# sash-a/CleanRL.jl

Measured on AMD Instinct MI355X. Metric: env-steps/sec (whole node), CartPole PPO num_envs=65536 at 1/2/4/8 GPUs, higher is better.
Workload: dtype f32 (64x64 products as fp16x2 split operands — hi + lo in f16, >= 22 significant bits — 3 f16 MFMAs per product, f32 accumulate; measured against a Float64 product on the headline's own operands this is as close as a plain f32 FMA chain: profiles/r06_product_error.json)

## Files before the change

### cleanrl.jl_amd/_lib.py

```python
import ctypes as C
import os

import numpy as np

_HERE = os.path.dirname(os.path.abspath(__file__))
LIB_PATH = os.environ.get("CRL_LIB_PATH") or os.path.join(_HERE, "libcleanrl_hip.so")


class CrlError(RuntimeError):
    pass


class CrlConfig(C.Structure):
    _fields_ = [
        ("total_timesteps", C.c_int64), ("num_steps", C.c_int32), ("num_envs", C.c_int32),
        ("num_minibatches", C.c_int32), ("update_epochs", C.c_int32), ("lr", C.c_float), ("gamma", C.c_float),
        ("gae_lambda", C.c_float), ("clip_coef", C.c_float), ("ent_coeff", C.c_float), ("v_coef", C.c_float),
        ("normalize_advantages", C.c_int32), ("clip_value_loss", C.c_int32), ("anneal_lr", C.c_int32),
        ("obs_dim", C.c_int32), ("n_act", C.c_int32), ("hidden", C.c_int32), ("gae_mode", C.c_int32),
        ("env_kind", C.c_int32), ("stale_obs", C.c_int32), ("env_id_offset", C.c_int32), ("shuffle_mode", C.c_int32),
        ("seed", C.c_uint64),
    ]


# ... 39 lines not shown
        return {n: getattr(self, n) for n, _ in self._fields_}


EXPORTS = [
    "crl_version", "crl_last_error", "crl_device_count", "crl_ppo_create", "crl_ppo_destroy", "crl_ppo_param_count",
    "crl_sync", "crl_ppo_write", "crl_ppo_read", "crl_policy_act", "crl_logprob_actions", "crl_gae",
    "crl_rollout_store", "crl_env_reset", "crl_rollout_run", "crl_episode_stats_read", "crl_compute_gae",
    "crl_shuffle", "crl_adv_stats", "crl_ppo_update_minibatch", "crl_ppo_iterate", "crl_ppo_iteration",
    "crl_comm_unique_id", "crl_comm_init", "crl_comm_init_external", "crl_comm_peer_export", "crl_comm_peer_attach", "crl_adv_stats_local", "crl_adv_stats_finish",
    "crl_prof_enable", "crl_prof_read", "crl_prof_reset", "crl_ppo_exact_reruns", "crl_episode_ring_enable",
    "crl_episode_ring_read", "crl_comm_destroy", "crl_ppo_set_option", "crl_ppo_get_option", "crl_ppo_option_name", "crl_ppo_option_count", "crl_gae_bench", "crl_gae_opt",
    "crl_a2c_create", "crl_a2c_destroy", "crl_a2c_param_count", "crl_a2c_write_params", "crl_a2c_read_params",
    "crl_a2c_read_env", "crl_a2c_read_buffer", "crl_a2c_run_until_update", "crl_a2c_discounted_future_rewards",
    "crl_dqn_create", "crl_dqn_destroy", "crl_dqn_write_params", "crl_dqn_read_params", "crl_dqn_status_read", "crl_dqn_run",
    "crl_dqn_q_values",
    "crl_make_actor_critic", "crl_ppo_init_params", "crl_a2c_init_params", "crl_dqn_make_nn", "crl_dqn_init_params", "crl_comm_info", "crl_clock_probe", "crl_product_probe", "crl_ppo_iterate_async", "crl_ppo_drain",
    "crl_env_step", "crl_ppo_evaluate", "crl_ppo_diagnose",
    "crl_ppo_stream", "crl_rollout_act_device", "crl_rollout_record_device", "crl_env_step_device", "crl_ppo_update",
]

DQN_PARAM_COUNT = 10934


class CrlDQNConfig(C.Structure):
    _fields_ = [("log_frequency", C.c_int64), ("total_timesteps", C.c_int64), ("buffer_size", C.c_int64), ("min_buff_size", C.c_int64),
                ("lr", C.c_double), ("train_freq", C.c_int64), ("target_net_freq", C.c_int64), ("batch_size", C.c_int64),
                ("gamma", C.c_double), ("epsilon_start", C.c_double), ("epsilon_end", C.c_double), ("epsilon_duration", C.c_double),
                ("max_steps", C.c_int32), ("pad", C.c_int32), ("seed", C.c_uint64)]


class CrlDQNEpisode(C.Structure):
# ... 109 lines not shown
    L.crl_make_actor_critic.argtypes = [C.c_int32, C.c_int32, C.c_int32, C.c_uint64, fp, C.c_size_t]
    L.crl_ppo_init_params.argtypes = [vp, C.c_uint64]
    L.crl_a2c_init_params.argtypes = [vp, C.c_uint64]
    L.crl_dqn_make_nn.argtypes = [C.c_uint64, fp, C.c_size_t]
    L.crl_dqn_init_params.argtypes = [vp, C.c_uint64]
    L.crl_comm_info.argtypes = [C.c_char_p, C.c_size_t, ip]
    L.crl_clock_probe.argtypes = [C.c_int32, C.c_double, dp, dp, dp]
    L.crl_ppo_iterate_async.argtypes = [vp, C.POINTER(CrlIterationReport), C.POINTER(CrlStats), C.POINTER(CrlEpisodeRecord), C.c_int32]
    L.crl_ppo_drain.argtypes = [vp, C.POINTER(CrlIterationReport), C.POINTER(CrlStats), C.POINTER(CrlEpisodeRecord), C.c_int32]
    L.crl_ppo_stream.argtypes = [vp, C.POINTER(vp)]
    L.crl_rollout_act_device.argtypes = [vp, C.c_int32, vp, vp, vp, vp]
    L.crl_rollout_record_device.argtypes = [vp, C.c_int32, vp, vp, vp, vp]
    L.crl_env_step_device.argtypes = [vp, vp, C.c_uint64, vp, vp, vp, vp]
    L.crl_ppo_update.argtypes = [vp, C.POINTER(CrlStats)]
    L.crl_product_probe.argtypes = [C.c_int32, C.c_int32, fp, fp, C.c_int32, C.c_int32, C.c_int32, C.c_int32, C.c_float, C.c_float, fp, fp]
    for name in EXPORTS:
        if name not in ("crl_version", "crl_last_error"):
            getattr(L, name).restype = C.c_int32
    _lib = L
    return L


def check(rc):
    if rc != 0:
        raise CrlError(load().crl_last_error().decode("utf-8", "replace"))


def device_count():
    n = C.c_int32(0)
    rc = load().crl_device_count(C.byref(n))
# ... 76 lines not shown
            self.close()
        except Exception:
            pass


def product_probe(flavour, A, B, chunks=1, scale_a=1.0, scale_b=1.0, col_scale=None, device=0):
    A = np.ascontiguousarray(A, np.float32); B = np.ascontiguousarray(B, np.float32)
    rows, K = A.shape; cols = B.shape[0]
    out = np.zeros((chunks, cols, rows), np.float32)
    cs = None if col_scale is None else np.ascontiguousarray(col_scale, np.float32)
    check(load().crl_product_probe(device, flavour, _ptr(A, C.c_float), _ptr(B, C.c_float), rows, cols, K, chunks, scale_a, scale_b,
                                   None if cs is None else _ptr(cs, C.c_float), _ptr(out, C.c_float)))
    return out


def clock_probe(device=0, span_ms=5.0):
    med, lo, hi = C.c_double(0), C.c_double(0), C.c_double(0)
    check(load().crl_clock_probe(device, span_ms, C.byref(med), C.byref(lo), C.byref(hi)))
    return med.value, lo.value, hi.value


def comm_info():
    buf = C.create_string_buffer(4096)
    ver = C.c_int32(0)
    check(load().crl_comm_info(buf, len(buf), C.byref(ver)))
    return buf.value.decode("utf-8", "replace"), int(ver.value)


def make_actor_critic_host(obs_dim, n_act, hidden, seed=0):
    n = 2 * (hidden * obs_dim + hidden + hidden * hidden + hidden) + n_act * hidden + n_act + hidden + 1
# ... 431 lines not shown
```

### cleanrl.jl_amd/csrc/mlp_x2.hpp

```cpp
#pragma once
#include "common.hpp"
#include "mlp_x3.hpp"

namespace crl {

typedef _Float16 f16x8 __attribute__((ext_vector_type(8)));
typedef _Float16 f16x2 __attribute__((ext_vector_type(2)));

constexpr float X2_ACT_SCALE = 16384.0f;
constexpr float X2_W_SCALE = 256.0f;
constexpr float X2_W_LIMIT = 255.0f;
constexpr float X2_W_SMALL = 0.00048828125f;
constexpr float X2_FWD_UNSCALE = 1.0f / (16384.0f * 256.0f);

struct P2 { f16x8 hi, lo; };

__device__ __forceinline__ P2 split2(const float (&x)[8]) {
  P2 p;
#pragma unroll
  for (int q = 0; q < 4; ++q) {
    f32x2 v; v[0] = x[2 * q]; v[1] = x[2 * q + 1];
    const f16x2 h = __builtin_convertvector(v, f16x2);
    f32x2 r;
    const uint32_t hb = __builtin_bit_cast(uint32_t, h);
    asm("v_fma_mix_f32 %0, %1, -1.0, %2 op_sel_hi:[1,0,0]" : "=v"(r[0]) : "v"(hb), "v"(v[0]));
    asm("v_fma_mix_f32 %0, %1, -1.0, %2 op_sel:[1,0,0] op_sel_hi:[1,0,0]" : "=v"(r[1]) : "v"(hb), "v"(v[1]));
    const f16x2 l = __builtin_convertvector(r, f16x2);
    p.hi[2 * q] = h[0]; p.hi[2 * q + 1] = h[1];
    p.lo[2 * q] = l[0]; p.lo[2 * q + 1] = l[1];
  }
  return p;
}

__device__ __forceinline__ f32x16 mfma_f16(f16x8 a, f16x8 b, f32x16 c) {
  return __builtin_amdgcn_mfma_f32_32x32x16_f16(a, b, c, 0, 0, 0);
}
__device__ __forceinline__ f32x16 mfma_x2(const P2& a, const P2& b, f32x16 c) {
  c = mfma_f16(a.lo, b.hi, c);
  c = mfma_f16(a.hi, b.lo, c);
  c = mfma_f16(a.hi, b.hi, c);
  return c;
}

template <int D, int NOUT, bool BWD = true>
struct NetImageX2 {
  static constexpr int PIECE = 2048;
  static constexpr int WF2H = 0;
  static constexpr int WB2H = WF2H + 2 * PIECE;
  static constexpr int WF1 = WB2H + (BWD ? 2 * PIECE : 0);
  static constexpr int B1C = WF1 + 2 * (D / 2) * 64;
  static constexpr int B2C = B1C + 64;
  static constexpr int W3 = B2C + 64;
  static constexpr int B3 = W3 + NOUT * 64;
  static constexpr int SIZE = ((B3 + NOUT + 3) / 4) * 4;
};

template <int D, int NOUT, bool BWD = true>
__device__ __forceinline__ bool stage_net_x2(float* img, const float* __restrict__ p, int tid, int nthreads, int* lds_flag) {
  using I = NetImageX2<D, NOUT, BWD>;
  using P = NetParams<D, NOUT>;
  _Float16* wf = reinterpret_cast<_Float16*>(img + I::WF2H);
  _Float16* wb = reinterpret_cast<_Float16*>(img + I::WB2H);
  if (tid == 0) *lds_flag = 0;
  __syncthreads();
  bool bad = false, big = false;
  for (int idx = tid; idx < 4096; idx += nthreads) {
    const int j = idx & 7, lane = (idx >> 3) & 63, ks = (idx >> 9) & 3, mo = idx >> 11;
    const int i = lane & 31, hf = lane >> 5;
    const int row = 32 * mo + i, k = kmap(ks, j, hf);
    {
      const float w0 = p[P::W2 + row + H * k];
      bad |= !(__builtin_fabsf(w0) < X2_W_LIMIT);
      big |= __builtin_fabsf(w0) >= X2_W_SMALL;
      const float w = w0 * X2_W_SCALE;
      const _Float16 h = (_Float16)w;
      wf[idx] = h; wf[4096 + idx] = (_Float16)(w - (float)h);
    }
    if (BWD) {
// ... 7 lines not shown
    int i = lane & 31, hf = lane >> 5;
    img[I::WF1 + idx] = p[P::W1 + (32 * mo + i) + H * (2 * ks + hf)] * TWO_LOG2E;
  }
  for (int idx = tid; idx < 64; idx += nthreads) {
    int r = idx & 15, mo = (idx >> 4) & 1, hf = idx >> 5;
    int row = 32 * mo + rowmap(r, hf);
    img[I::B1C + idx] = p[P::B1 + row] * TWO_LOG2E;
    img[I::B2C + idx] = p[P::B2 + row] * (X2_ACT_SCALE * X2_W_SCALE);
  }
  for (int idx = tid; idx < NOUT * 64; idx += nthreads) {
    int q = idx & 31, hf = (idx >> 5) & 1, a = idx >> 6;
    int mt = q >> 4, r = q & 15;
    img[I::W3 + idx] = p[P::W3 + a + NOUT * (32 * mt + rowmap(r, hf))];
  }
  for (int idx = tid; idx < NOUT; idx += nthreads) img[I::B3 + idx] = p[P::B3 + idx];
  if (bad) atomicOr(lds_flag, 1);
  if (big) atomicOr(lds_flag, 2);
  __syncthreads();
  return *lds_flag == 2;
}

__device__ __forceinline__ P2 load_wfrag2(const float* piece0, int mo, int ks, int lane) {
  const f16x8* q = reinterpret_cast<const f16x8*>(piece0) + ((mo * 4 + ks) * 64 + lane);
  P2 a;
  a.hi = q[0]; a.lo = q[512];
  return a;
}

__device__ __forceinline__ void dense64_x2(const float* wimg, const f32x16 (&xs)[2], f32x16& acc0, f32x16& acc1, int lane) {
#pragma unroll
  for (int ks = 0; ks < 4; ++ks) {
    float xb[8];
#pragma unroll
    for (int j = 0; j < 8; ++j) xb[j] = xs[ks >> 1][8 * (ks & 1) + j];
    const P2 b = split2(xb);
    acc0 = mfma_x2(load_wfrag2(wimg, 0, ks, lane), b, acc0);
    acc1 = mfma_x2(load_wfrag2(wimg, 1, ks, lane), b, acc1);
  }
}

template <int D, int NOUT, bool BWD = true>
__device__ __forceinline__ void mlp_forward_x2(const float* img, const float (&x)[D], f32x16 (&h1s)[2], f32x16 (&h2)[2],
                                               float (&out)[NOUT], int lane) {
  using I = NetImageX2<D, NOUT, BWD>;
  const int hf = lane >> 5;
  f32x16 a0 = load16(img + I::B1C + hf * 32);
  f32x16 a1 = load16(img + I::B1C + hf * 32 + 16);
#pragma unroll
  for (int ks = 0; ks < D / 2; ++ks) {
    const float b = hf ? x[2 * ks + 1] : x[2 * ks];
    a0 = mfma32(img[I::WF1 + (0 * (D / 2) + ks) * 64 + lane], b, a0);
    a1 = mfma32(img[I::WF1 + (1 * (D / 2) + ks) * 64 + lane], b, a1);
  }
#pragma unroll
  for (int r = 0; r < 16; ++r) { h1s[0][r] = tanh_exp2_arg(a0[r], X2_ACT_SCALE); h1s[1][r] = tanh_exp2_arg(a1[r], X2_ACT_SCALE); }
  a0 = load16(img + I::B2C + hf * 32);
  a1 = load16(img + I::B2C + hf * 32 + 16);
  dense64_x2(img + I::WF2H, h1s, a0, a1, lane);
#pragma unroll
  for (int r = 0; r < 16; ++r) {
    h2[0][r] = tanh_exp2(a0[r], TWO_LOG2E * X2_FWD_UNSCALE, 1.0f); h2[1][r] = tanh_exp2(a1[r], TWO_LOG2E * X2_FWD_UNSCALE, 1.0f);
  }
#pragma unroll
  for (int a = 0; a < NOUT; ++a) {
    const f32x4* w = reinterpret_cast<const f32x4*>(img + I::W3 + a * 64 + hf * 32);
    float acc = 0.0f;
#pragma unroll
    for (int q = 0; q < 8; ++q) {
// ... 47 lines not shown
```

### cleanrl.jl_amd/csrc/policy.hip

```cpp
#include <cstdlib>

#include "common.hpp"
#include "env.hpp"
#include "mlp_x3.hpp"
#include "mlp_x2.hpp"
#include "ppo_ctx.hpp"
#include "rollout_env.hpp"

namespace crl {

template <int D, int A>
__global__ void __launch_bounds__(256) policy_act_kernel(const float* __restrict__ params, const float* __restrict__ obs,
                                                         const double* __restrict__ u, int n, int32_t* __restrict__ action,
                                                         float* __restrict__ logprob, float* __restrict__ value) {
  using IA = NetImage<D, A, false>;
  extern __shared__ __attribute__((aligned(16))) float smem[];
  float* imgA = smem;
  float* imgC = smem + IA::SIZE;
  stage_net<D, A, false>(imgA, params, threadIdx.x, blockDim.x);
  stage_net<D, 1, false>(imgC, params + NetParams<D, A>::SIZE, threadIdx.x, blockDim.x);
  __syncthreads();
  const int lane = threadIdx.x & 63, wave = threadIdx.x >> 6, j = lane & 31, hf = lane >> 5;
  const int wpb = blockDim.x >> 6;
  for (int tile = blockIdx.x * wpb + wave; tile * TILE < n; tile += gridDim.x * wpb) {
// ... 164 lines not shown
  using L = RolloutLds1<A>;
  extern __shared__ __attribute__((aligned(16))) float smem[];
  float* imgA0 = smem + L::IMG_A;
  float* imgC0 = smem + L::IMG_C;
  bool cx2 = CX2;
  stage_net_x3<D, A, false>(imgA0, a.params, threadIdx.x, blockDim.x);
  if (CX2) {
    int* flag = reinterpret_cast<int*>(smem + L::FLAG);
    if (!stage_net_x2<D, 1, false>(imgC0, a.params + NetParams<D, A>::SIZE, threadIdx.x, blockDim.x, flag)) {
      if (threadIdx.x == 0 && blockIdx.x == 0) a.range_err[0] = 1.0;
      cx2 = false;
    }
  }
  if (!cx2) stage_net_x3<D, 1, false>(imgC0, a.params + NetParams<D, A>::SIZE, threadIdx.x, blockDim.x);
  __syncthreads();
  const DevCfg& c = a.c;
  const int lane = threadIdx.x & 63, wave = threadIdx.x >> 6, j = lane & 31, hf = lane >> 5;
  const int wpb = blockDim.x >> 6;
  const int e = (blockIdx.x * wpb + wave) * TILE + j;
  const bool ok = e < c.nt;
  const bool writer = ok && hf == 0;
  const int ee = ok ? e : 0;
  const uint32_t gid = c.env_id_offset + (uint32_t)ee;

  EnvOwner env;
  env_owner_load(env, a, ee);

  if (__builtin_amdgcn_readfirstlane(wave) >= 4) {
    for (int i = 0; i < a.stagger; ++i) __builtin_amdgcn_s_sleep(16);
  }

  for (int step = 0; step < c.k; ++step) {
    const uint64_t gstep = a.iteration * (uint64_t)c.k + (uint64_t)step;
    const size_t b = (size_t)ee + (size_t)c.nt * step;
    f32x16 h1[2], h2[2];
    float z[A], v[1];
    int lds_off = 0;
    asm volatile("" : "+v"(lds_off));
    const float* imgA = imgA0 + lds_off;
    const float* imgC = imgC0 + lds_off;
    const float cx[4] = {env.co[0], env.co[1], env.co[2], env.co[3]};
    mlp_forward_x3<D, A, false>(imgA, cx, h1, h2, z, lane);
    float lpa;
    const int act = env_owner_sample<A>(z, u53(philox_env(c.seed, gid, gstep, 0)), lpa);
    if (CX2 && cx2) mlp_forward_x2<D, 1, false>(imgC, cx, h1, h2, v, lane);
    else mlp_forward_x3<D, 1, false>(imgC, cx, h1, h2, v, lane);
    if (writer) a.value[b] = v[0];
    env_owner_advance(env, a, act, lpa, gid, gstep, step, b, writer);
  }
  if (writer) env_owner_store(env, a, e);
  if (a.fuse_gae) {
    __builtin_amdgcn_fence(__ATOMIC_RELEASE, "workgroup");
    __builtin_amdgcn_fence(__ATOMIC_ACQUIRE, "workgroup");
  }
  env_owner_finish(env, a, e, writer);
}

template <int A>
__global__ void __launch_bounds__(128) rollout_split_kernel(RolloutArgs a) {
  constexpr int D = 4;
// ... 68 lines not shown
  }
  const DevCfg& c = a.c;
  const int lane = threadIdx.x & 63, wave = __builtin_amdgcn_readfirstlane(threadIdx.x >> 6), j = lane & 31, hf = lane >> 5;
  const int e = blockIdx.x * TILE + j;
  const bool ok = e < c.nt;
  const bool writer = ok && hf == 0;
  const int ee = ok ? e : 0;
  const uint32_t gid = c.env_id_offset + (uint32_t)ee;

  EnvOwner env;
  if (wave == 1) {
    env_owner_load(env, a, ee);
    if (hf == 0) xch[j] = make_float4(env.co[0], env.co[1], env.co[2], env.co[3]);
  }
  __syncthreads();

  for (int step = 0; step < c.k; ++step) {
    const uint64_t gstep = a.iteration * (uint64_t)c.k + (uint64_t)step;
    const size_t b = (size_t)ee + (size_t)c.nt * step;
    int lds_off = 0;
    asm volatile("" : "+v"(lds_off));
    if (wave < 2) {
      const int mo = wave;
      const float* img = imgA0 + lds_off;
      float cx[4];
      if (wave == 1) { cx[0] = env.co[0]; cx[1] = env.co[1]; cx[2] = env.co[2]; cx[3] = env.co[3]; }
      else { const float4 cv = xch[(step & 1) * TILE + j]; cx[0] = cv.x; cx[1] = cv.y; cx[2] = cv.z; cx[3] = cv.w; }
      double u = 0.0;
      if (wave == 1) u = u53(philox_env(c.seed, gid, gstep, 0));
      f32x16 acc = layer1_rows32<IA>(img, cx, mo, lane);
// ... 39 lines not shown
        if (hf == 0) xch[((step + 1) & 1) * TILE + j] = make_float4(env.co[0], env.co[1], env.co[2], env.co[3]);
      }
    } else if (!cx2) {
      const float4 cv = xch[(step & 1) * TILE + j];
      const float cx[4] = {cv.x, cv.y, cv.z, cv.w};
      f32x16 h1[2], h2[2];
      float v[1];
      mlp_forward_x3<D, 1, false>(imgC0 + lds_off, cx, h1, h2, v, lane);
      __syncthreads();
      __syncthreads();
      if (writer) a.value[b] = v[0];
    } else {
      const float* img = imgC0 + lds_off;
      const float4 cv = xch[(step & 1) * TILE + j];
      const float cx[4] = {cv.x, cv.y, cv.z, cv.w};
      f32x16 a0 = layer1_rows32<IC>(img, cx, 0, lane), a1 = layer1_rows32<IC>(img, cx, 1, lane);
      f32x16 h1s[2];
#pragma unroll
      for (int r = 0; r < 16; ++r) { h1s[0][r] = tanh_exp2_arg(a0[r], X2_ACT_SCALE); h1s[1][r] = tanh_exp2_arg(a1[r], X2_ACT_SCALE); }
      __syncthreads();
      a0 = load16(img + IC::B2C + hf * 32); a1 = load16(img + IC::B2C + hf * 32 + 16);
      dense64_x2(img + IC::WF2H, h1s, a0, a1, lane);
      const f32x4* w = reinterpret_cast<const f32x4*>(img + IC::W3 + hf * 32);
      float accv = 0.0f;
#pragma unroll
      for (int q = 0; q < 8; ++q) {
        const f32x4 wv = w[q];
#pragma unroll
        for (int i = 0; i < 4; ++i) {
          const int idx = q * 4 + i;
          const float hv = tanh_exp2((idx >> 4) ? a1[idx & 15] : a0[idx & 15], TWO_LOG2E * X2_FWD_UNSCALE, 1.0f);
// ... 124 lines not shown
  using IA = NetImageA16<A>;
  using L = RolloutLds6<A>;
  extern __shared__ __attribute__((aligned(16))) float smem[];
  float* imgA0 = smem + L::IMG_A;
  float* imgC0 = smem + L::IMG_C;
  float* xch = smem + L::XCH;
  uint2* pcsA = reinterpret_cast<uint2*>(smem + L::PCS_A);
  float* pcsC = smem + L::PCS_C;
  float* hdA = smem + L::HD_A;
  float* hdC = smem + L::HD_C;
  double* ubuf = reinterpret_cast<double*>(smem + L::UBUF);
  float4* rbuf = reinterpret_cast<float4*>(smem + L::RBUF);
  int* flag = reinterpret_cast<int*>(smem + L::FLAG);
  stage_net_a16<A>(imgA0, a.params, threadIdx.x, blockDim.x);
  bool cx2 = true;
  if (!stage_net_x2<D, 1, false>(imgC0, a.params + NetParams<D, A>::SIZE, threadIdx.x, blockDim.x, flag)) {
    if (threadIdx.x == 0 && blockIdx.x == 0) a.range_err[0] = 1.0;
    cx2 = false;
    stage_net_x3<D, 1, false>(imgC0, a.params + NetParams<D, A>::SIZE, threadIdx.x, blockDim.x);
  }
  const DevCfg& c = a.c;
  const int lane = threadIdx.x & 63, wave = __builtin_amdgcn_readfirstlane(threadIdx.x >> 6);
  const int e = blockIdx.x * TILE + (lane & 31);
  const bool envlane = wave == 0 && lane < 32;
  const bool ok = e < c.nt;
  const bool writer = ok && envlane;
  const int ee = ok ? e : 0;
  const uint32_t gid = c.env_id_offset + (uint32_t)ee;
  EnvOwner env;
  if (envlane) {
    env_owner_load(env, a, ee);
// ... 230 lines not shown
```

### cleanrl.jl_amd/csrc/probe.hip

```cpp
#include <hip/hip_runtime.h>

#include <algorithm>
#include <string>
#include <vector>

#include "ppo_ctx.hpp"

namespace crl {
__global__ void __launch_bounds__(512) clock_probe_kernel(long long span_ticks, double* __restrict__ mhz, float* __restrict__ sink) {
  float a0 = threadIdx.x * 1e-3f, a1 = 1.0f, a2 = 2.0f, a3 = 3.0f, a4 = 4.0f, a5 = 5.0f, a6 = 6.0f, a7 = 7.0f;
  const float m = 0.999f, c = 1e-3f;
  const long long w0 = wall_clock64();
  const unsigned long long c0 = __builtin_readcyclecounter();
  long long w1 = w0;
  do {
#pragma unroll 1
    for (int i = 0; i < 256; ++i) {
      a0 = __builtin_fmaf(a0, m, c); a1 = __builtin_fmaf(a1, m, c); a2 = __builtin_fmaf(a2, m, c); a3 = __builtin_fmaf(a3, m, c);
      a4 = __builtin_fmaf(a4, m, c); a5 = __builtin_fmaf(a5, m, c); a6 = __builtin_fmaf(a6, m, c); a7 = __builtin_fmaf(a7, m, c);
    }
    w1 = wall_clock64();
  } while (w1 - w0 < span_ticks);
  const unsigned long long c1 = __builtin_readcyclecounter();
  if ((threadIdx.x & 63) == 0) mhz[blockIdx.x * (blockDim.x >> 6) + (threadIdx.x >> 6)] = (double)(c1 - c0) / ((double)(w1 - w0) / 100.0);
// ... 52 lines not shown
      float a[8], b[8];
#pragma unroll
      for (int j = 0; j < 8; ++j) {
        a[j] = A[(size_t)row * K + k0 + k + 8 * hf + j];
        b[j] = B[(size_t)col * K + k0 + k + 8 * hf + j];
        if constexpr (FLAVOUR == 0) { a[j] *= sa; b[j] *= sbc; }
      }
      if constexpr (FLAVOUR == 0) acc = mfma_x2(split2(a), split2(b), acc);
      else acc = mfma_x3(split3(a), split3(b), acc);
    }
  }
  float un = 1.0f;
  if constexpr (FLAVOUR == 0) un = 1.0f / (sa * sbc);
  for (int r = 0; r < 16; ++r) C[((size_t)ch * cols + col) * rows + 32 * rt + rowmap(r, hf)] = acc[r] * un;
}
}

extern "C" int32_t crl_product_probe(int32_t device, int32_t flavour, const float* A, const float* B, int32_t rows, int32_t cols, int32_t K, int32_t chunks,
                                     float scale_a, float scale_b, const float* col_scale, float* C) {
  using namespace crl;
  if (!A || !B || !C || rows <= 0 || cols <= 0 || K <= 0 || chunks <= 0 || rows % 32 || cols % 32 || K % chunks || (K / chunks) % 16 || flavour < 0 || flavour > 3) {
    set_error("crl_product_probe: rows / cols multiples of 32, K / chunks a multiple of 16, flavour 0 … 3"); return 1;
  }
  CRL_HIP_CHECK(hipSetDevice(device));
  const size_t na = (size_t)rows * K, nb = (size_t)cols * K, nc = (size_t)chunks * rows * cols;
  float *dA = nullptr, *dB = nullptr, *dC = nullptr, *dS = nullptr;
  int rc = 0;
  auto fail = [&](hipError_t e, const char* what) { set_error(std::string("crl_product_probe: ") + what + ": " + hipGetErrorString(e)); rc = 1; };
  hipError_t e;
  if ((e = hipMalloc(reinterpret_cast<void**>(&dA), na * 4)) != hipSuccess) fail(e, "hipMalloc");
  if (!rc && (e = hipMalloc(reinterpret_cast<void**>(&dB), nb * 4)) != hipSuccess) fail(e, "hipMalloc");
  if (!rc && (e = hipMalloc(reinterpret_cast<void**>(&dC), nc * 4)) != hipSuccess) fail(e, "hipMalloc");
  if (!rc && col_scale && (e = hipMalloc(reinterpret_cast<void**>(&dS), (size_t)cols * 4)) != hipSuccess) fail(e, "hipMalloc");
  if (!rc && (e = hipMemcpy(dA, A, na * 4, hipMemcpyHostToDevice)) != hipSuccess) fail(e, "copy A");
  if (!rc && (e = hipMemcpy(dB, B, nb * 4, hipMemcpyHostToDevice)) != hipSuccess) fail(e, "copy B");
  if (!rc && col_scale && (e = hipMemcpy(dS, col_scale, (size_t)cols * 4, hipMemcpyHostToDevice)) != hipSuccess) fail(e, "copy scales");
  if (!rc) {
    const dim3 grid(rows / 32, cols / 32, chunks), block(64);
    const int kc = K / chunks;
    switch (flavour) {
      case 0: hipLaunchKernelGGL(product_probe_kernel<0>, grid, block, 0, 0, dA, dB, rows, cols, K, kc, scale_a, scale_b, dS, dC); break;
      case 1: hipLaunchKernelGGL(product_probe_kernel<1>, grid, block, 0, 0, dA, dB, rows, cols, K, kc, scale_a, scale_b, dS, dC); break;
      case 2: hipLaunchKernelGGL(product_probe_kernel<2>, grid, block, 0, 0, dA, dB, rows, cols, K, kc, scale_a, scale_b, dS, dC); break;
      default: hipLaunchKernelGGL(product_probe_kernel<3>, grid, block, 0, 0, dA, dB, rows, cols, K, kc, scale_a, scale_b, dS, dC); break;
    }
    if ((e = hipGetLastError()) != hipSuccess) fail(e, "launch");
    if (!rc && (e = hipMemcpy(C, dC, nc * 4, hipMemcpyDeviceToHost)) != hipSuccess) fail(e, "copy C");
  }
  (void)hipFree(dA); (void)hipFree(dB); (void)hipFree(dC); (void)hipFree(dS);
  return rc;
}
```

### cleanrl.jl_amd/csrc/update.hip

```cpp
#include <hip/hip_ext.h>

#include <cstdlib>

#include "common.hpp"
#include "mlp_x2.hpp"
#include "mlp_x3.hpp"
#include "ppo_ctx.hpp"
#include "stats.hpp"
#include "update_args.hpp"

namespace crl {

#ifdef CRL_EXP_STAMPS
__device__ unsigned long long crl_dbg_stamps[512 * 8 * 8];
#define CRL_STAMP(slot) do { if ((threadIdx.x & 63) == 0) crl_dbg_stamps[((size_t)blockIdx.x * 8 + (threadIdx.x >> 6)) * 8 + (slot)] = wall_clock64(); } while (0)
__device__ unsigned crl_dbg_tstamps[512 * 8 * 16];
#ifndef CRL_TS_SET
#define CRL_TS_SET 0
#endif
constexpr int crl_ts_slot(int k) { return k == 0 ? 0 : k == 9 ? 5 : (CRL_TS_SET == 0 ? (k <= 4 ? k : -1) : (k >= 5 ? k - 4 : -1)); }
#define CRL_TS(k) do { if constexpr (crl_ts_slot(k) >= 0) { if (ts_on) ts[crl_ts_slot(k)] = (unsigned)__builtin_amdgcn_s_memrealtime(); } } while (0)
#else
#define CRL_STAMP(slot) do { } while (0)
#define CRL_TS(k) do { } while (0)
// ... 67 lines not shown
  constexpr int NT = 64 * RW;
  float* img0 = smem;
  float* T0 = scratch + wave * SCR;
  const float* p = a.params + (ROLE ? NetParams<D, A>::SIZE : 0);
  CRL_STAMP(0);
  if constexpr (X2) {
    if (!stage_net_x2<D, NOUT>(img0, p, tid, NT, reinterpret_cast<int*>(scratch + RW * SCR))) {
      if (tid == 0 && rb == 0) a.range_err[0] = 1.0;
      __syncthreads();
      return false;
    }
  }
  else if (X3) stage_net_x3<D, NOUT, true>(img0, p, tid, NT);
  else stage_net<D, NOUT, true>(img0, p, tid, NT);
  __syncthreads();

  CRL_STAMP(1);
  f32x16 dW2t[2][2];
#pragma unroll
  for (int x = 0; x < 2; ++x)
#pragma unroll
    for (int y = 0; y < 2; ++y)
#pragma unroll
      for (int r = 0; r < 16; ++r) dW2t[x][y][r] = 0.0f;
  constexpr int K_B1 = D, K_B2 = D + 1, K_W3 = D + 2, K_B3 = D + 2 + NOUT, NACC = D + 2 + 2 * NOUT;
  float racc[NACC];
#pragma unroll
  for (int i = 0; i < NACC; ++i) racc[i] = 0.0f;
  float* ACC = scratch + wave * SCR + SCR_FLOATS + (threadIdx.x & 63);
  if constexpr (X3) {
#pragma unroll
    for (int i = 0; i < NACC; ++i) ACC[64 * i] = 0.0f;
  }
  constexpr bool LACC = X3;
  auto acc_begin = [&](int k) -> float { if constexpr (LACC) return ACC[64 * k]; else return racc[k]; };
  auto acc_end = [&](int k, float v) { if constexpr (LACC) ACC[64 * k] = v; else racc[k] = v; };
  double ls0 = 0.0, ls1 = 0.0;

  const int M = c.M;
  const int ntiles = (M + TILE - 1) / TILE;
  const int nwaves = a.nblk[ROLE] * RW;
  const double invM = X2 ? sgpr_hard(1.0 / a.Mglobal) : sgpr(1.0 / a.Mglobal);
  float mean_f = 0.0f; double inv_denom = 1.0;
  if (ROLE == 0) {
    mean_f = sgpr((float)a.adv_ms[2 * a.mb]);
    const double idn = 1.0 / ((double)(float)a.adv_ms[2 * a.mb + 1] + 1e-8);
    inv_denom = X2 ? sgpr_hard(idn) : sgpr(idn);
  }
  const float eps = c.clip, lo = 1.0f - c.clip, hi = 1.0f + c.clip;
  const float u_exact = EXACT ? sgpr((float)a.vfix[0]) : 0.0f;
  const double nwin = EXACT ? sgpr(a.vfix[1]) : 0.0;
  const double entk0 = (double)c.ent_coeff / ((double)A * a.Mglobal), vk0 = (double)c.v_coef * 0.5 * invM;
  const double entk = X2 ? sgpr_hard(entk0) : sgpr(entk0);
  const double vk = X2 ? sgpr_hard(vk0) : sgpr(vk0);

  int tile = rb * RW + wave, tstride = nwaves;
  if (a.xcd_align) {
    const int gx = rb & 7;
    tile = gx + 8 * ((rb >> 3) * RW + wave);
    tstride = 8 * (a.nblk[ROLE] >> 3) * RW;
  }
  Gathered<D> cur;
  constexpr bool PF = ((X2 && ABL == 0) || (X3 && ABL == 128 && CRL_PF_X3 != 0)) && !EXACT && CRL_PF_ENABLED != 0;
  const f32x4* pf4 = nullptr;
  const int* pfi = nullptr;
  unsigned pf_lds = 0;
  auto pos_of = [&](int t) { const int p = t * TILE + j; return p < M ? p : 0; };
// ... 61 lines not shown
      const int d = __builtin_amdgcn_readfirstlane(tile - partner_tile), half = tstride >> 1;
      if (d < -half) __builtin_amdgcn_s_setprio(3); else if (d < half && (wave >> 2)) __builtin_amdgcn_s_setprio(1); else __builtin_amdgcn_s_setprio(0);
    }
    CRL_TS(1);
    float x[D];
#pragma unroll
    for (int i = 0; i < D; ++i) x[i] = cur.x[i];
    f32x16 h1[2], h2[2];
    float out[NOUT], dout[NOUT];
    int lds_off = 0;
    asm volatile("" : "+v"(lds_off));
    const float* img = img0 + lds_off;
    float* T = T0 + lds_off;
    float* xs = T + 64 * TSTRIDE;
    float* d3s = xs + TILE * D;
    if constexpr (X2) mlp_forward_x2<D, NOUT>(img, x, h1, h2, out, lane);
    else if constexpr (X3) mlp_forward_x3<D, NOUT, true, ABL>(img, x, h1, h2, out, lane);
    else mlp_forward<D, NOUT, true>(img, x, h1, h2, out, lane);
    CRL_TS(2);

    if constexpr ((ABL & 32) != 0) {
#pragma unroll
      for (int i = 0; i < NOUT; ++i) dout[i] = out[i] * 1e-6f + cur.f0 + cur.f1 + (float)cur.act;
    } else if constexpr (ROLE == 0) {
      float pr[A], lp[A];
      softmax_logsoftmax<A>(out, pr, lp);
      const int act = cur.act;
      float nlp = lp[0];
#pragma unroll
      for (int i = 1; i < A; ++i) nlp = (act == i) ? lp[i] : nlp;
      double Hs = 0.0;
// ... 913 lines not shown
```

### include/cleanrl_hip.h

```cpp
#ifndef CLEANRL_HIP_H
#define CLEANRL_HIP_H
#include <stddef.h>
#include <stdint.h>

#ifdef __cplusplus
extern "C" {
#endif

#define CRL_VERSION 100

#define CRL_GAE_COMPAT 0
#define CRL_GAE_FIXED 1
#define CRL_ENV_CARTPOLE 0
#define CRL_ENV_SYNTHETIC 1
#define CRL_ENV_EXTERNAL 2
#define CRL_ENV_MOUNTAINCAR 3
#define CRL_ENV_ACROBOT 4
#define CRL_SHUFFLE_FISHER_YATES 0
#define CRL_SHUFFLE_BIJECTION 1
#define CRL_SHUFFLE_BLOCKED_FY 2
enum crl_field {
  CRL_F_OBS = 0,
  CRL_F_ACTION = 1,
  CRL_F_LOGPROB = 2,
// ... 135 lines not shown
int32_t crl_comm_destroy(crl_ppo* h);

int32_t crl_ppo_set_option(crl_ppo* h, const char* key, int64_t value);
int32_t crl_ppo_get_option(crl_ppo* h, const char* key, int64_t* value);
int32_t crl_ppo_option_name(int32_t index, const char** name, int64_t* dflt);
int32_t crl_ppo_option_count(int32_t* n);

enum crl_kernel_id { CRL_K_ROLLOUT = 0, CRL_K_GAE = 1, CRL_K_SHUFFLE = 2, CRL_K_ADV_STATS = 3, CRL_K_UPDATE = 4,
                     CRL_K_REDUCE = 5, CRL_K_OPTIM = 6, CRL_K_ALLREDUCE = 7, CRL_K_PACK = 8, CRL_K_PERMUTE = 9,
                     CRL_K_COUNT = 10 };
int32_t crl_gae_bench(int32_t device, int32_t nt, int32_t k, int32_t seg, int32_t tile, int32_t nt_loads, int32_t flush_mb,
                      int32_t reps, double* gae_ms, double* copy_ms);
int32_t crl_clock_probe(int32_t device, double span_ms, double* median_mhz, double* min_mhz, double* max_mhz);
int32_t crl_product_probe(int32_t device, int32_t flavour, const float* A, const float* B, int32_t rows, int32_t cols, int32_t K, int32_t chunks,
                          float scale_a, float scale_b, const float* col_scale, float* C);
int32_t crl_prof_enable(crl_ppo* h, int32_t on);
int32_t crl_prof_read(crl_ppo* h, int32_t kernel_id, double* total_ms, int64_t* launches);
int32_t crl_prof_reset(crl_ppo* h);

typedef struct crl_a2c_config {
  double lr;
  int64_t total_timesteps;
  int32_t min_replay_size;
  int32_t max_steps;
  double gamma;
  uint64_t seed;
} crl_a2c_config;
typedef struct crl_a2c_train_stats { double actor_loss, critic_loss; int32_t n, trained; } crl_a2c_train_stats;
typedef struct crl_a2c_episode { double episode_return; int64_t episode_length, global_step; } crl_a2c_episode;
typedef struct crl_a2c crl_a2c;
// ... 45 lines not shown
```

Measured before the change: 836.3 million.

## Compute critic layer 1 with split-f16 MFMA folding bias into the product

Replaces the fp32 MFMA path for the critic's first layer (4 observations plus bias) with a single 16-wide f16 MFMA per 32-row block. Weights are staged once into LDS as hi/lo f16 pieces with the bias folded in as an extra K slot, and observations are split into hi/lo at runtime. A per-block weight-magnitude check and a per-wave ballot on input range fall back to the old fp32 path when values would overflow or lose precision. The intent is to cut the layer-1 MFMA count and drop the bias accumulator load, at the cost of extra staging work, larger LDS images and a runtime branch. It also adds probe entry points for checking accuracy.

```diff
diff --git a/cleanrl.jl_amd/_lib.py b/cleanrl.jl_amd/_lib.py
--- a/cleanrl.jl_amd/_lib.py
+++ b/cleanrl.jl_amd/_lib.py
@@ -77,7 +77,7 @@
     "crl_a2c_read_env", "crl_a2c_read_buffer", "crl_a2c_run_until_update", "crl_a2c_discounted_future_rewards",
     "crl_dqn_create", "crl_dqn_destroy", "crl_dqn_write_params", "crl_dqn_read_params", "crl_dqn_status_read", "crl_dqn_run",
     "crl_dqn_q_values",
-    "crl_make_actor_critic", "crl_ppo_init_params", "crl_a2c_init_params", "crl_dqn_make_nn", "crl_dqn_init_params", "crl_comm_info", "crl_clock_probe", "crl_product_probe", "crl_ppo_iterate_async", "crl_ppo_drain",
+    "crl_make_actor_critic", "crl_ppo_init_params", "crl_a2c_init_params", "crl_dqn_make_nn", "crl_dqn_init_params", "crl_comm_info", "crl_clock_probe", "crl_product_probe", "crl_layer1_f16_slots", "crl_ppo_iterate_async", "crl_ppo_drain",
     "crl_env_step", "crl_ppo_evaluate", "crl_ppo_diagnose",
     "crl_ppo_stream", "crl_rollout_act_device", "crl_rollout_record_device", "crl_env_step_device", "crl_ppo_update",
 ]
@@ -217,6 +217,7 @@
     L.crl_env_step_device.argtypes = [vp, vp, C.c_uint64, vp, vp, vp, vp]
     L.crl_ppo_update.argtypes = [vp, C.POINTER(CrlStats)]
     L.crl_product_probe.argtypes = [C.c_int32, C.c_int32, fp, fp, C.c_int32, C.c_int32, C.c_int32, C.c_int32, C.c_float, C.c_float, fp, fp]
+    L.crl_layer1_f16_slots.argtypes = [ip]
     for name in EXPORTS:
         if name not in ("crl_version", "crl_last_error"):
             getattr(L, name).restype = C.c_int32
@@ -323,6 +324,12 @@
     return out
 
 
+def layer1_f16_slots():
+    out = np.zeros((64, 8, 3), np.int32)
+    check(load().crl_layer1_f16_slots(_ptr(out, C.c_int32)))
+    return out
+
+
 def clock_probe(device=0, span_ms=5.0):
     med, lo, hi = C.c_double(0), C.c_double(0), C.c_double(0)
     check(load().crl_clock_probe(device, span_ms, C.byref(med), C.byref(lo), C.byref(hi)))
diff --git a/cleanrl.jl_amd/csrc/layer1_f16.hpp b/cleanrl.jl_amd/csrc/layer1_f16.hpp
--- /dev/null
+++ b/cleanrl.jl_amd/csrc/layer1_f16.hpp
@@ -0,0 +1,19 @@
+#pragma once
+
+namespace crl {
+
+enum L1Piece : int { L1_ZERO = 0, L1_HI = 1, L1_LO = 2, L1_BIAS_HI = 3, L1_BIAS_LO = 4, L1_ONE = 5 };
+struct L1Slot { int a, b, c; };
+
+constexpr int L1_SLOTS = 16;
+constexpr L1Slot layer1_f16_slot(int k) {
+  return k < 4 ? L1Slot{L1_HI, L1_HI, k}
+       : k < 8 ? L1Slot{L1_HI, L1_LO, k - 4}
+       : k < 12 ? L1Slot{L1_LO, L1_HI, k - 8}
+       : k == 12 ? L1Slot{L1_BIAS_HI, L1_ONE, 0}
+       : k == 13 ? L1Slot{L1_BIAS_LO, L1_ONE, 0}
+       : L1Slot{L1_ZERO, L1_ZERO, 0};
+}
+constexpr int layer1_f16_k(int lane, int j) { return 8 * (lane >> 5) + j; }
+
+}
diff --git a/cleanrl.jl_amd/csrc/mlp_x2.hpp b/cleanrl.jl_amd/csrc/mlp_x2.hpp
--- a/cleanrl.jl_amd/csrc/mlp_x2.hpp
+++ b/cleanrl.jl_amd/csrc/mlp_x2.hpp
@@ -1,5 +1,6 @@
 #pragma once
 #include "common.hpp"
+#include "layer1_f16.hpp"
 #include "mlp_x3.hpp"
 
 namespace crl {
@@ -12,20 +13,27 @@
 constexpr float X2_W_LIMIT = 255.0f;
 constexpr float X2_W_SMALL = 0.00048828125f;
 constexpr float X2_FWD_UNSCALE = 1.0f / (16384.0f * 256.0f);
+constexpr float X2_L1_LIMIT = 32768.0f;
+constexpr float X2_L1_SMALL = 0.125f;
+constexpr float X2_L1_TERM = 128.0f;
 
 struct P2 { f16x8 hi, lo; };
 
+__device__ __forceinline__ void split2_pair(f32x2 v, f16x2& h, f16x2& l) {
+  h = __builtin_convertvector(v, f16x2);
+  f32x2 r;
+  const uint32_t hb = __builtin_bit_cast(uint32_t, h);
+  asm("v_fma_mix_f32 %0, %1, -1.0, %2 op_sel_hi:[1,0,0]" : "=v"(r[0]) : "v"(hb), "v"(v[0]));
+  asm("v_fma_mix_f32 %0, %1, -1.0, %2 op_sel:[1,0,0] op_sel_hi:[1,0,0]" : "=v"(r[1]) : "v"(hb), "v"(v[1]));
+  l = __builtin_convertvector(r, f16x2);
+}
 __device__ __forceinline__ P2 split2(const float (&x)[8]) {
   P2 p;
 #pragma unroll
   for (int q = 0; q < 4; ++q) {
     f32x2 v; v[0] = x[2 * q]; v[1] = x[2 * q + 1];
-    const f16x2 h = __builtin_convertvector(v, f16x2);
-    f32x2 r;
-    const uint32_t hb = __builtin_bit_cast(uint32_t, h);
-    asm("v_fma_mix_f32 %0, %1, -1.0, %2 op_sel_hi:[1,0,0]" : "=v"(r[0]) : "v"(hb), "v"(v[0]));
-    asm("v_fma_mix_f32 %0, %1, -1.0, %2 op_sel:[1,0,0] op_sel_hi:[1,0,0]" : "=v"(r[1]) : "v"(hb), "v"(v[1]));
-    const f16x2 l = __builtin_convertvector(r, f16x2);
+    f16x2 h, l;
+    split2_pair(v, h, l);
     p.hi[2 * q] = h[0]; p.hi[2 * q + 1] = h[1];
     p.lo[2 * q] = l[0]; p.lo[2 * q + 1] = l[1];
   }
@@ -52,16 +60,18 @@
   static constexpr int B2C = B1C + 64;
   static constexpr int W3 = B2C + 64;
   static constexpr int B3 = W3 + NOUT * 64;
-  static constexpr int SIZE = ((B3 + NOUT + 3) / 4) * 4;
+  static constexpr int A1F = ((B3 + NOUT + 3) / 4) * 4;
+  static constexpr int L1WMAX = A1F + 2 * 64 * 4;
+  static constexpr int SIZE = L1WMAX + 4;
 };
 
-template <int D, int NOUT, bool BWD = true>
+template <int D, int NOUT, bool BWD = true, bool L1F = true>
 __device__ __forceinline__ bool stage_net_x2(float* img, const float* __restrict__ p, int tid, int nthreads, int* lds_flag) {
   using I = NetImageX2<D, NOUT, BWD>;
   using P = NetParams<D, NOUT>;
   _Float16* wf = reinterpret_cast<_Float16*>(img + I::WF2H);
   _Float16* wb = reinterpret_cast<_Float16*>(img + I::WB2H);
-  if (tid == 0) *lds_flag = 0;
+  if (tid == 0) { *lds_flag = 0; if (L1F) img[I::L1WMAX] = 0.0f; }
   __syncthreads();
   bool bad = false, big = false;
   for (int idx = tid; idx < 4096; idx += nthreads) {
@@ -99,8 +109,25 @@
     img[I::W3 + idx] = p[P::W3 + a + NOUT * (32 * mt + rowmap(r, hf))];
   }
   for (int idx = tid; idx < NOUT; idx += nthreads) img[I::B3 + idx] = p[P::B3 + idx];
+  static_assert(D == 4, "the slot table of layer1_f16.hpp is laid out for four observations");
+  _Float16* a1f = reinterpret_cast<_Float16*>(img + I::A1F);
+  bool bad1 = false;
+  float wmax1 = 0.0f;
+  for (int idx = tid; L1F && idx < 2 * 64 * 8; idx += nthreads) {
+    const int j = idx & 7, lane = (idx >> 3) & 63, mo = idx >> 9;
+    const int row = 32 * mo + (lane & 31);
+    const L1Slot s = layer1_f16_slot(layer1_f16_k(lane, j));
+    const bool bias = s.a == L1_BIAS_HI || s.a == L1_BIAS_LO;
+    float w = 0.0f;
+    if (s.a != L1_ZERO) w = __fmul_rn(bias ? p[P::B1 + row] : p[P::W1 + row + H * s.c], TWO_LOG2E);
+    bad1 |= !(__builtin_fabsf(w) < X2_L1_LIMIT);
+    if (!bias) wmax1 = __builtin_fmaxf(wmax1, __builtin_fabsf(w));
+    const _Float16 h = (_Float16)w;
+    a1f[idx] = (s.a == L1_LO || s.a == L1_BIAS_LO) ? (_Float16)(w - (float)h) : h;
+  }
   if (bad) atomicOr(lds_flag, 1);
   if (big) atomicOr(lds_flag, 2);
+  if (L1F) atomicMax(reinterpret_cast<unsigned*>(img + I::L1WMAX), bad1 ? 0x7F800000u : __float_as_uint(wmax1));
   __syncthreads();
   return *lds_flag == 2;
 }
@@ -124,19 +151,59 @@
   }
 }
 
+template <class I>
+__device__ __forceinline__ float layer1_limit(const float* img0) {
+  const float wm = __uint_as_float((unsigned)__builtin_amdgcn_readfirstlane((int)__float_as_uint(img0[I::L1WMAX])));
+  return (wm >= X2_L1_SMALL && wm < X2_L1_LIMIT) ? X2_L1_TERM / wm : 0.0f;
+}
+template <class I, int D>
+__device__ __forceinline__ void layer1_x2(const float* img, const float (&x)[D], f32x16& a0, f32x16& a1, int lane, float l1lim, float xsmall = X2_L1_SMALL) {
+  static_assert(D == 4, "the slot table of layer1_f16.hpp is laid out for four observations");
+  const int hf = lane >> 5;
+  bool xbad = false;
+  float xmax = 0.0f;
+#pragma unroll
+  for (int c = 0; c < D; ++c) { xbad |= !(__builtin_fabsf(x[c]) < l1lim); xmax = __builtin_fmaxf(xmax, __builtin_fabsf(x[c])); }
+  if (__builtin_amdgcn_ballot_w64(xbad) == 0 && __builtin_amdgcn_ballot_w64(xmax >= xsmall) != 0) {
+    f16x2 xh[2], xl[2];
+#pragma unroll
+    for (int q = 0; q < 2; ++q) { f32x2 v; v[0] = x[2 * q]; v[1] = x[2 * q + 1]; split2_pair(v, xh[q], xl[q]); }
+    const auto piece = [&](int k) -> _Float16 {
+      const L1Slot s = layer1_f16_slot(k);
+      return s.b == L1_HI ? xh[s.c >> 1][s.c & 1] : s.b == L1_LO ? xl[s.c >> 1][s.c & 1] : s.b == L1_ONE ? (_Float16)1.0f : (_Float16)0.0f;
+    };
+    u32x4v bw;
+#pragma unroll
+    for (int q = 0; q < 4; ++q) {
+      f16x2 lo2, hi2;
+      lo2[0] = piece(2 * q); lo2[1] = piece(2 * q + 1);
+      hi2[0] = piece(8 + 2 * q); hi2[1] = piece(8 + 2 * q + 1);
+      bw[q] = hf ? __builtin_bit_cast(uint32_t, hi2) : __builtin_bit_cast(uint32_t, lo2);
+    }
+    const f16x8 b = __builtin_bit_cast(f16x8, bw);
+    const f16x8* af = reinterpret_cast<const f16x8*>(img + I::A1F) + lane;
+    const f32x16 zero = {};
+    a0 = mfma_f16(af[0], b, zero);
+    a1 = mfma_f16(af[64], b, zero);
+  } else {
+    a0 = load16(img + I::B1C + hf * 32);
+    a1 = load16(img + I::B1C + hf * 32 + 16);
+#pragma unroll
+    for (int ks = 0; ks < D / 2; ++ks) {
+      const float b = hf ? x[2 * ks + 1] : x[2 * ks];
+      a0 = mfma32(img[I::WF1 + (0 * (D / 2) + ks) * 64 + lane], b, a0);
+      a1 = mfma32(img[I::WF1 + (1 * (D / 2) + ks) * 64 + lane], b, a1);
+    }
+  }
+}
+
 template <int D, int NOUT, bool BWD = true>
 __device__ __forceinline__ void mlp_forward_x2(const float* img, const float (&x)[D], f32x16 (&h1s)[2], f32x16 (&h2)[2],
-                                               float (&out)[NOUT], int lane) {
+                                               float (&out)[NOUT], int lane, float l1lim) {
   using I = NetImageX2<D, NOUT, BWD>;
   const int hf = lane >> 5;
-  f32x16 a0 = load16(img + I::B1C + hf * 32);
-  f32x16 a1 = load16(img + I::B1C + hf * 32 + 16);
-#pragma unroll
-  for (int ks = 0; ks < D / 2; ++ks) {
-    const float b = hf ? x[2 * ks + 1] : x[2 * ks];
-    a0 = mfma32(img[I::WF1 + (0 * (D / 2) + ks) * 64 + lane], b, a0);
-    a1 = mfma32(img[I::WF1 + (1 * (D / 2) + ks) * 64 + lane], b, a1);
-  }
+  f32x16 a0, a1;
+  layer1_x2<I>(img, x, a0, a1, lane, l1lim);
 #pragma unroll
   for (int r = 0; r < 16; ++r) { h1s[0][r] = tanh_exp2_arg(a0[r], X2_ACT_SCALE); h1s[1][r] = tanh_exp2_arg(a1[r], X2_ACT_SCALE); }
   a0 = load16(img + I::B2C + hf * 32);
diff --git a/cleanrl.jl_amd/csrc/policy.hip b/cleanrl.jl_amd/csrc/policy.hip
--- a/cleanrl.jl_amd/csrc/policy.hip
+++ b/cleanrl.jl_amd/csrc/policy.hip
@@ -202,6 +202,7 @@
   }
   if (!cx2) stage_net_x3<D, 1, false>(imgC0, a.params + NetParams<D, A>::SIZE, threadIdx.x, blockDim.x);
   __syncthreads();
+  const float l1lim = (CX2 && cx2) ? layer1_limit<NetImageX2<D, 1, false>>(imgC0) : 0.0f;
   const DevCfg& c = a.c;
   const int lane = threadIdx.x & 63, wave = threadIdx.x >> 6, j = lane & 31, hf = lane >> 5;
   const int wpb = blockDim.x >> 6;
@@ -231,7 +232,7 @@
     mlp_forward_x3<D, A, false>(imgA, cx, h1, h2, z, lane);
     float lpa;
     const int act = env_owner_sample<A>(z, u53(philox_env(c.seed, gid, gstep, 0)), lpa);
-    if (CX2 && cx2) mlp_forward_x2<D, 1, false>(imgC, cx, h1, h2, v, lane);
+    if (CX2 && cx2) mlp_forward_x2<D, 1, false>(imgC, cx, h1, h2, v, lane, l1lim);
     else mlp_forward_x3<D, 1, false>(imgC, cx, h1, h2, v, lane);
     if (writer) a.value[b] = v[0];
     env_owner_advance(env, a, act, lpa, gid, gstep, step, b, writer);
@@ -330,6 +331,7 @@
     if (hf == 0) xch[j] = make_float4(env.co[0], env.co[1], env.co[2], env.co[3]);
   }
   __syncthreads();
+  const float l1lim = cx2 ? layer1_limit<IC>(imgC0) : 0.0f;
 
   for (int step = 0; step < c.k; ++step) {
     const uint64_t gstep = a.iteration * (uint64_t)c.k + (uint64_t)step;
@@ -399,7 +401,8 @@
       const float* img = imgC0 + lds_off;
       const float4 cv = xch[(step & 1) * TILE + j];
       const float cx[4] = {cv.x, cv.y, cv.z, cv.w};
-      f32x16 a0 = layer1_rows32<IC>(img, cx, 0, lane), a1 = layer1_rows32<IC>(img, cx, 1, lane);
+      f32x16 a0, a1;
+      layer1_x2<IC>(img, cx, a0, a1, lane, l1lim);
       f32x16 h1s[2];
 #pragma unroll
       for (int r = 0; r < 16; ++r) { h1s[0][r] = tanh_exp2_arg(a0[r], X2_ACT_SCALE); h1s[1][r] = tanh_exp2_arg(a1[r], X2_ACT_SCALE); }
@@ -554,7 +557,7 @@
   int* flag = reinterpret_cast<int*>(smem + L::FLAG);
   stage_net_a16<A>(imgA0, a.params, threadIdx.x, blockDim.x);
   bool cx2 = true;
-  if (!stage_net_x2<D, 1, false>(imgC0, a.params + NetParams<D, A>::SIZE, threadIdx.x, blockDim.x, flag)) {
+  if (!stage_net_x2<D, 1, false, false>(imgC0, a.params + NetParams<D, A>::SIZE, threadIdx.x, blockDim.x, flag)) {
     if (threadIdx.x == 0 && blockIdx.x == 0) a.range_err[0] = 1.0;
     cx2 = false;
     stage_net_x3<D, 1, false>(imgC0, a.params + NetParams<D, A>::SIZE, threadIdx.x, blockDim.x);
diff --git a/cleanrl.jl_amd/csrc/probe.hip b/cleanrl.jl_amd/csrc/probe.hip
--- a/cleanrl.jl_amd/csrc/probe.hip
+++ b/cleanrl.jl_amd/csrc/probe.hip
@@ -90,13 +90,51 @@
   if constexpr (FLAVOUR == 0) un = 1.0f / (sa * sbc);
   for (int r = 0; r < 16; ++r) C[((size_t)ch * cols + col) * rows + 32 * rt + rowmap(r, hf)] = acc[r] * un;
 }
+
+template <int MODE>
+__global__ void __launch_bounds__(64) layer1_probe_kernel(const float* __restrict__ A, const float* __restrict__ B, float* __restrict__ C) {
+  using I = NetImageX2<4, 1, false>;
+  using P = NetParams<4, 1>;
+  __shared__ __attribute__((aligned(16))) float img[I::SIZE];
+  __shared__ float par[P::SIZE];
+  __shared__ int flag;
+  const int lane = threadIdx.x, hf = lane >> 5, col = 32 * blockIdx.x + (lane & 31);
+  for (int i = lane; i < P::SIZE; i += 64) par[i] = 0.0f;
+  __syncthreads();
+  for (int c = 0; c < 4; ++c) par[P::W1 + lane + H * c] = A[lane * 5 + c];
+  par[P::B1 + lane] = A[lane * 5 + 4];
+  __syncthreads();
+  stage_net_x2<4, 1, false>(img, par, lane, 64, &flag);
+  __syncthreads();
+  const float l1lim = MODE == 0 ? layer1_limit<I>(img) : MODE == 1 ? 0.0f : X2_L1_LIMIT;
+  const float x[4] = {B[col * 5 + 0], B[col * 5 + 1], B[col * 5 + 2], B[col * 5 + 3]};
+  f32x16 a0, a1;
+  layer1_x2<I>(img, x, a0, a1, lane, l1lim, MODE == 2 ? 0.0f : X2_L1_SMALL);
+  for (int r = 0; r < 16; ++r) { C[(size_t)col * 64 + rowmap(r, hf)] = a0[r]; C[(size_t)col * 64 + 32 + rowmap(r, hf)] = a1[r]; }
+}
+}
+
+extern "C" int32_t crl_layer1_f16_slots(int32_t* out) {
+  using namespace crl;
+  if (!out) { set_error("crl_layer1_f16_slots: out must hold 64 x 8 x 3 values"); return 1; }
+  for (int lane = 0; lane < 64; ++lane)
+    for (int j = 0; j < 8; ++j) {
+      const L1Slot s = layer1_f16_slot(layer1_f16_k(lane, j));
+      int32_t* q = out + (lane * 8 + j) * 3;
+      q[0] = s.a; q[1] = s.b; q[2] = s.c;
+    }
+  return 0;
 }
 
 extern "C" int32_t crl_product_probe(int32_t device, int32_t flavour, const float* A, const float* B, int32_t rows, int32_t cols, int32_t K, int32_t chunks,
                                      float scale_a, float scale_b, const float* col_scale, float* C) {
   using namespace crl;
-  if (!A || !B || !C || rows <= 0 || cols <= 0 || K <= 0 || chunks <= 0 || rows % 32 || cols % 32 || K % chunks || (K / chunks) % 16 || flavour < 0 || flavour > 3) {
-    set_error("crl_product_probe: rows / cols multiples of 32, K / chunks a multiple of 16, flavour 0 … 3"); return 1;
+  const bool layer1 = flavour >= 4 && flavour <= 6;
+  if (layer1 && (!A || !B || !C || rows != 64 || cols <= 0 || cols % 32 || K != 5 || chunks != 1)) {
+    set_error("crl_product_probe: flavours 4 … 6 take rows = 64, K = 5 (W1 row + b1 | x + unused), chunks = 1, cols a multiple of 32"); return 1;
+  }
+  if (!layer1 && (!A || !B || !C || rows <= 0 || cols <= 0 || K <= 0 || chunks <= 0 || rows % 32 || cols % 32 || K % chunks || (K / chunks) % 16 || flavour < 0 || flavour > 3)) {
+    set_error("crl_product_probe: rows / cols multiples of 32, K / chunks a multiple of 16, flavour 0 … 6"); return 1;
   }
   CRL_HIP_CHECK(hipSetDevice(device));
   const size_t na = (size_t)rows * K, nb = (size_t)cols * K, nc = (size_t)chunks * rows * cols;
@@ -115,6 +153,9 @@
     const dim3 grid(rows / 32, cols / 32, chunks), block(64);
     const int kc = K / chunks;
     switch (flavour) {
+      case 4: hipLaunchKernelGGL(layer1_probe_kernel<0>, dim3(cols / 32), block, 0, 0, dA, dB, dC); break;
+      case 5: hipLaunchKernelGGL(layer1_probe_kernel<1>, dim3(cols / 32), block, 0, 0, dA, dB, dC); break;
+      case 6: hipLaunchKernelGGL(layer1_probe_kernel<2>, dim3(cols / 32), block, 0, 0, dA, dB, dC); break;
       case 0: hipLaunchKernelGGL(product_probe_kernel<0>, grid, block, 0, 0, dA, dB, rows, cols, K, kc, scale_a, scale_b, dS, dC); break;
       case 1: hipLaunchKernelGGL(product_probe_kernel<1>, grid, block, 0, 0, dA, dB, rows, cols, K, kc, scale_a, scale_b, dS, dC); break;
       case 2: hipLaunchKernelGGL(product_probe_kernel<2>, grid, block, 0, 0, dA, dB, rows, cols, K, kc, scale_a, scale_b, dS, dC); break;
diff --git a/cleanrl.jl_amd/csrc/update.hip b/cleanrl.jl_amd/csrc/update.hip
--- a/cleanrl.jl_amd/csrc/update.hip
+++ b/cleanrl.jl_amd/csrc/update.hip
@@ -105,6 +105,8 @@
   else if (X3) stage_net_x3<D, NOUT, true>(img0, p, tid, NT);
   else stage_net<D, NOUT, true>(img0, p, tid, NT);
   __syncthreads();
+  float l1lim = 0.0f;
+  if constexpr (X2) l1lim = layer1_limit<I>(img0);
 
   CRL_STAMP(1);
   f32x16 dW2t[2][2];
@@ -131,7 +133,9 @@
   const int M = c.M;
   const int ntiles = (M + TILE - 1) / TILE;
   const int nwaves = a.nblk[ROLE] * RW;
-  const double invM = X2 ? sgpr_hard(1.0 / a.Mglobal) : sgpr(1.0 / a.Mglobal);
+  double Mg = a.Mglobal;
+  if constexpr (X2) asm volatile("" : "+s"(Mg));
+  const double invM = X2 ? sgpr_hard(1.0 / Mg) : sgpr(1.0 / Mg);
   float mean_f = 0.0f; double inv_denom = 1.0;
   if (ROLE == 0) {
     mean_f = sgpr((float)a.adv_ms[2 * a.mb]);
@@ -141,7 +145,7 @@
   const float eps = c.clip, lo = 1.0f - c.clip, hi = 1.0f + c.clip;
   const float u_exact = EXACT ? sgpr((float)a.vfix[0]) : 0.0f;
   const double nwin = EXACT ? sgpr(a.vfix[1]) : 0.0;
-  const double entk0 = (double)c.ent_coeff / ((double)A * a.Mglobal), vk0 = (double)c.v_coef * 0.5 * invM;
+  const double entk0 = (double)c.ent_coeff / ((double)A * Mg), vk0 = (double)c.v_coef * 0.5 * invM;
   const double entk = X2 ? sgpr_hard(entk0) : sgpr(entk0);
   const double vk = X2 ? sgpr_hard(vk0) : sgpr(vk0);
 
@@ -233,7 +237,7 @@
     float* T = T0 + lds_off;
     float* xs = T + 64 * TSTRIDE;
     float* d3s = xs + TILE * D;
-    if constexpr (X2) mlp_forward_x2<D, NOUT>(img, x, h1, h2, out, lane);
+    if constexpr (X2) mlp_forward_x2<D, NOUT>(img, x, h1, h2, out, lane, l1lim);
     else if constexpr (X3) mlp_forward_x3<D, NOUT, true, ABL>(img, x, h1, h2, out, lane);
     else mlp_forward<D, NOUT, true>(img, x, h1, h2, out, lane);
     CRL_TS(2);
diff --git a/include/cleanrl_hip.h b/include/cleanrl_hip.h
--- a/include/cleanrl_hip.h
+++ b/include/cleanrl_hip.h
@@ -173,6 +173,7 @@
 int32_t crl_clock_probe(int32_t device, double span_ms, double* median_mhz, double* min_mhz, double* max_mhz);
 int32_t crl_product_probe(int32_t device, int32_t flavour, const float* A, const float* B, int32_t rows, int32_t cols, int32_t K, int32_t chunks,
                           float scale_a, float scale_b, const float* col_scale, float* C);
+int32_t crl_layer1_f16_slots(int32_t* out);
 int32_t crl_prof_enable(crl_ppo* h, int32_t on);
 int32_t crl_prof_read(crl_ppo* h, int32_t kernel_id, double* total_ms, int64_t* launches);
 int32_t crl_prof_reset(crl_ppo* h);
```

After: 842.8 million, median of 6. About the same (+0.8%).
